# gaozhitong/MultiShiftSeg

Measured on AMD Instinct MI355X. Metric: train images/sec (DeepLabV3+ WRN38, fwd + RelContrastiveLoss + bwd + Adam), higher is better.
Workload: dtype f32; 1 GPU; c3: 2 images (1 orig+aug pair(s)) of 1024x2048 per GPU, stage-2 trainable set, train-mode BN/Dropout2d on the frozen trunk; images_per_gpu=2, height=1024, width=2048, stage=2, parallelism=dp1, rccl_ranks=0, loss_pairing=device, loss_sync=local

## Files before the change

multishiftseg_amd/csrc/conv_igemm.hip:

```cpp
#include "mss_epilogue.h"
#include <stdlib.h>

#include "fwd_route.h"

int mss_gemm_nt_launch(MssConvArgs p, const FwdRoute& r, void* stream);
int mss_fwd_bf16x3_launch(MssConvArgs p, const FwdRoute& r, void* stream);
int mss_stem7_launch(MssConvArgs p, void* stream);
int mss_conv_dgrad_s2_launch(MssConvArgs p, const FwdRoute& r, void* stream);

namespace {

constexpr int NT = 256;

template <int BM, int BN, int BK, int WM, int WN, bool PER_SAMPLE, bool AFFINE>
__global__ __launch_bounds__(NT) void conv_igemm_kernel(MssConvArgs p) {
  constexpr int LDK = BK + 4;
  constexpr int WTM = BM / WM, WTN = BN / WN;
  constexpr int TM = WTM / 32, TN = WTN / 32;
  constexpr int CPR = BK / 4;
  constexpr int RPP = NT / CPR;
  constexpr int A_LD = BM / RPP, B_LD = BN / RPP;
  static_assert(WM * WN == 4, "4 waves per workgroup");
  static_assert(A_LD >= 1 && B_LD >= 1, "tile too small for 256 threads");

  extern __shared__ __attribute__((aligned(16))) float smem[];
  int* live_mask_p = reinterpret_cast<int*>(smem);
  float* As = smem + 4;
  float* Bs = As + 2 * BM * LDK;

  const int tid = threadIdx.x;
  const int lane = tid & 63;
  const int wave = tid >> 6;
  const int wm = wave / WN, wn = wave % WN;

  p.x += (size_t)blockIdx.y * p.x_bs;
  p.w += (size_t)blockIdx.y * p.w_bs;
  p.y += (size_t)blockIdx.y * p.y_bs;
  const int v = mss_xcd_remap(blockIdx.x, gridDim.x);
  const int mt = v / p.ntiles, nt = v % p.ntiles;
  const int m0 = mt * BM, n0 = nt * BN;

  const int chunk = tid % CPR;
  const int row0 = tid / CPR;

  int a_nb[A_LD], a_iy0[A_LD], a_ix0[A_LD], a_n[A_LD];
  const int ohw = p.OH * p.OW;
  int my_live = 0;
  if (tid == 0) *live_mask_p = 0;
#pragma unroll
  for (int j = 0; j < A_LD; ++j) {
    int m = m0 + row0 + j * RPP;
    if (m < p.M) {
      int n = m / ohw, rem = m - n * ohw;
      int oy = rem / p.OW, ox = rem - oy * p.OW;
      a_n[j] = n;
      a_nb[j] = n * p.H * p.W;
      a_iy0[j] = oy * p.stride - p.pad;
      a_ix0[j] = ox * p.stride - p.pad;
      for (int t = 0; t < p.R * p.S; ++t) {
        int iy = a_iy0[j] + (t / p.S) * p.dil, ix = a_ix0[j] + (t % p.S) * p.dil;
        if ((unsigned)iy < (unsigned)p.H && (unsigned)ix < (unsigned)p.W) my_live |= 1 << t;
      }
    } else {
      a_n[j] = 0; a_nb[j] = 0; a_iy0[j] = -0x40000000; a_ix0[j] = -0x40000000;
    }
  }
  __syncthreads();
  if (my_live) atomicOr(live_mask_p, my_live);
  __syncthreads();
  const int live = *live_mask_p;
  const int nlive = __popc(live);
  const int cblocks = p.C / BK;
  const int n_it = nlive * cblocks;

  f32x16 acc[TM][TN];
#pragma unroll
  for (int i = 0; i < TM; ++i)
#pragma unroll
    for (int j = 0; j < TN; ++j)
#pragma unroll
      for (int r = 0; r < 16; ++r) acc[i][j][r] = 0.f;

  constexpr int S_LD = 1;
  f32x4 areg[A_LD], breg[B_LD], sreg[S_LD], hreg[S_LD];
  const float* a_ptr[A_LD];
  const float* b_ptr[B_LD];
  const float* s_ptr[S_LD];
  const float* h_ptr[S_LD];
  unsigned a_ok = 0;
  unsigned ld_ok = 0;
  int ld_cc = 0;
  int ld_tap = -1, ld_c0 = 0, ld_left = live;
  constexpr bool has_affine = AFFINE;
  const float relu_floor = p.in_relu ? 0.f : -__builtin_huge_valf();

  auto next_tap = [&]() {
    ld_tap = __ffs(ld_left) - 1;
    ld_left &= ld_left - 1;
    ld_c0 = 0;
    const int r = ld_tap / p.S, s = ld_tap - r * p.S;
    const int dy = r * p.dil, dx = s * p.dil;
    a_ok = 0;
#pragma unroll
    for (int j = 0; j < A_LD; ++j) {
      const int iy = a_iy0[j] + dy, ix = a_ix0[j] + dx;
      const bool ok = (unsigned)iy < (unsigned)p.H && (unsigned)ix < (unsigned)p.W;
      a_ok |= (ok ? 1u : 0u) << j;
      a_ptr[j] = ok ? p.x + (size_t)(a_nb[j] + iy * p.W + ix) * p.ldx + chunk * 4 : p.x;
    }
#pragma unroll
    for (int j = 0; j < B_LD; ++j)
      b_ptr[j] = p.w + ((size_t)ld_tap * p.Kpad + n0 + row0 + j * RPP) * p.C + chunk * 4;
    if (has_affine) {
#pragma unroll
      for (int j = 0; j < S_LD; ++j) {
        const size_t so = (size_t)(m0 / ohw) * p.in_ss_stride + chunk * 4;
        s_ptr[j] = p.in_scale + so;
        h_ptr[j] = p.in_shift + so;
      }
    }
  };

  auto issue_loads = [&]() {
#pragma unroll
    for (int j = 0; j < A_LD; ++j) areg[j] = *reinterpret_cast<const f32x4*>(a_ptr[j]);
#pragma unroll
    for (int j = 0; j < B_LD; ++j) breg[j] = *reinterpret_cast<const f32x4*>(b_ptr[j]);
    if (has_affine) {
#pragma unroll
      for (int j = 0; j < S_LD; ++j) {
        sreg[j] = *reinterpret_cast<const f32x4*>(s_ptr[j]);
        hreg[j] = *reinterpret_cast<const f32x4*>(h_ptr[j]);
      }
    }
    ld_cc = ld_c0 + chunk * 4;
    ld_ok = a_ok;
  };
  auto advance = [&]() {
    if (ld_c0 + BK >= p.C) {
      if (ld_left) next_tap();
    } else {
      ld_c0 += BK;
#pragma unroll
      for (int j = 0; j < A_LD; ++j)
        if ((a_ok >> j) & 1) a_ptr[j] += BK;
#pragma unroll
      for (int j = 0; j < B_LD; ++j) b_ptr[j] += BK;
      if (has_affine) {
#pragma unroll
        for (int j = 0; j < S_LD; ++j) { s_ptr[j] += BK; h_ptr[j] += BK; }
      }
    }
  };

  auto finish_store = [&](int buf) {
#pragma unroll
    for (int j = 0; j < A_LD; ++j) {
      f32x4 val = areg[j];
      if (has_affine) {
        if (PER_SAMPLE) {
          const size_t so = (size_t)a_n[j] * p.in_ss_stride + ld_cc;
          val = val * *reinterpret_cast<const f32x4*>(p.in_scale + so) + *reinterpret_cast<const f32x4*>(p.in_shift + so);
        } else {
          val = val * sreg[0] + hreg[0];
        }
      }
      val.x = fmaxf(val.x, relu_floor); val.y = fmaxf(val.y, relu_floor);
      val.z = fmaxf(val.z, relu_floor); val.w = fmaxf(val.w, relu_floor);
      if (!((ld_ok >> j) & 1)) val = f32x4{0.f, 0.f, 0.f, 0.f};
      *reinterpret_cast<f32x4*>(&As[(buf * BM + row0 + j * RPP) * LDK + chunk * 4]) = val;
    }
#pragma unroll
    for (int j = 0; j < B_LD; ++j)
      *reinterpret_cast<f32x4*>(&Bs[(buf * BN + row0 + j * RPP) * LDK + chunk * 4]) = breg[j];
  };

  if (n_it > 0) {
    next_tap();
    issue_loads();
    finish_store(0);
    advance();
    issue_loads();
    advance();
  }
  __syncthreads();

  constexpr int NKC = BK / 8;
  const int frag_row = lane & 31, frag_k = (lane >> 5) * 4;
  const float* Abase = &As[(wm * WTM + frag_row) * LDK + frag_k];
  const float* Bbase = &Bs[(wn * WTN + frag_row) * LDK + frag_k];
  f32x4 fa[2][TM], fb[2][TN];
  auto load_frags = [&](int set, int buf, int kc) {
#pragma unroll
    for (int i = 0; i < TM; ++i)
      fa[set][i] = *reinterpret_cast<const f32x4*>(Abase + (buf * BM + i * 32) * LDK + kc * 8);
#pragma unroll
    for (int j = 0; j < TN; ++j)
      fb[set][j] = *reinterpret_cast<const f32x4*>(Bbase + (buf * BN + j * 32) * LDK + kc * 8);
  };
  auto mfma_chunk = [&](int set) {
#pragma unroll
    for (int s = 0; s < 4; ++s)
#pragma unroll
      for (int i = 0; i < TM; ++i)
#pragma unroll
        for (int j = 0; j < TN; ++j)
          acc[i][j] = __builtin_amdgcn_mfma_f32_32x32x2f32(fa[set][i][s], fb[set][j][s], acc[i][j], 0, 0, 0);
  };

  if (n_it > 0) load_frags(0, 0, 0);
  for (int it = 0; it < n_it; ++it) {
    const int buf = it & 1;
#pragma unroll
    for (int kc = 0; kc < NKC; ++kc) {
      if (kc + 1 < NKC) load_frags((kc + 1) & 1, buf, kc + 1);
      if (kc == NKC - 2) { finish_store(buf ^ 1); issue_loads(); advance(); }
      if (kc == NKC - 1) {
        __syncthreads();
        load_frags(NKC & 1, buf ^ 1, 0);
      }
      mfma_chunk(kc & 1);
    }
  }

  mss_epilogue_store<TM, TN>(acc, p, p.y, m0 + wm * WTM, n0 + wn * WTN, lane);
}

template <int BM, int BN, int BK, int WM, int WN, bool PS, bool AFF>
int launch_conv_t(const MssConvArgs& p, hipStream_t stream) {
  const size_t smem = ((size_t)2 * (BM + BN) * (BK + 4) + 4) * sizeof(float);
  constexpr auto kern = conv_igemm_kernel<BM, BN, BK, WM, WN, PS, AFF>;
  if (int rc = mss_kernel_info<kern>(NT, smem)) return rc;
  hipLaunchKernelGGL(kern, dim3(p.mtiles * p.ntiles, p.batch > 1 ? p.batch : 1), dim3(NT), smem, stream, p);
  return mss_launch_status();
}

template <int BM, int BN, int BK, int WM, int WN>
int launch_conv_tile(const MssConvArgs& p, const FwdRoute& r, hipStream_t stream) {
  if (!r.affine) return launch_conv_t<BM, BN, BK, WM, WN, false, false>(p, stream);
  return r.per_sample ? launch_conv_t<BM, BN, BK, WM, WN, true, true>(p, stream) : launch_conv_t<BM, BN, BK, WM, WN, false, true>(p, stream);
}
int launch_conv(const MssConvArgs& p, const FwdRoute& r, hipStream_t stream) {
  if (r.BN == 64) return launch_conv_tile<256, 64, 16, 4, 1>(p, r, stream);
  return r.BK == 32 ? launch_conv_tile<128, 128, 32, 2, 2>(p, r, stream) : launch_conv_tile<128, 128, 16, 2, 2>(p, r, stream);
}

__global__ void pack_weights_kernel(const float* __restrict__ src, float* __restrict__ dst, int K, int C,
                                    int R, int S, int Kpad, int Cp, int flip, const int* __restrict__ col, int n_img, int c0) {
  const size_t total = (size_t)R * S * Kpad * Cp;
  for (size_t i = blockIdx.x * (size_t)blockDim.x + threadIdx.x; i < total;
       i += (size_t)gridDim.x * blockDim.x) {
    int c = i % Cp;
    int k = (i / Cp) % Kpad;
    int t = i / ((size_t)Cp * Kpad);
    int r = t / S, s = t % S;
    float val = 0.f;
    if (col) {
      if (k < K && c < C)
        for (int n = 0; n < n_img; ++n) {
          const int cc = c < c0 ? c : col[(size_t)n * (C - c0) + c - c0];
          if (cc >= 0) val += src[((((size_t)n * K + k) * C + (c < c0 ? c : c0 + cc)) * R + r) * S + s];
        }
    } else if (!flip) {
      if (k < K && c < C) val = src[(((size_t)k * C + c) * R + r) * S + s];
    } else {
      if (k < C && c < K) val = src[(((size_t)c * C + k) * R + (R - 1 - r)) * S + (S - 1 - s)];
    }
    dst[i] = val;
  }
}

__global__ void unpack_wgrad_kernel(const float* __restrict__ src, float* __restrict__ dst, int K, int C,
                                    int R, int S, int Kpad, int Cp, int accumulate, const int* __restrict__ place,
                                    const int* __restrict__ k_steps, int n_img, int c0) {
  if (place) {
    const size_t per = (size_t)K * C * R * S, all = per * n_img;
    for (size_t i = blockIdx.x * (size_t)blockDim.x + threadIdx.x; i < all; i += (size_t)gridDim.x * blockDim.x) {
      const size_t e = i % per;
      const int n = (int)(i / per);
      const int s = e % S, r = (e / S) % R;
      const int cc = (e / ((size_t)S * R)) % C, k = e / ((size_t)S * R * C);
      int c = cc;
      if (cc >= c0) {
        const int pc = cc - c0 < 16 * k_steps[n] ? place[(size_t)n * (C - c0) + cc - c0] : -1;
        c = pc >= 0 ? c0 + pc : -1;
      }
      dst[i] = c >= 0 ? src[((size_t)(r * S + s) * Kpad + k) * Cp + c] : 0.f;
    }
    return;
  }
  const size_t total = (size_t)K * C * R * S;
  for (size_t i = blockIdx.x * (size_t)blockDim.x + threadIdx.x; i < total;
       i += (size_t)gridDim.x * blockDim.x) {
    int s = i % S;
    int r = (i / S) % R;
    int c = (i / ((size_t)S * R)) % C;
    int k = i / ((size_t)S * R * C);
    float val = src[((size_t)(r * S + s) * Kpad + k) * Cp + c];
    dst[i] = accumulate ? dst[i] + val : val;
  }
}

constexpr int WP_CH = 128;
constexpr int WP_MIN_C = 32;
constexpr int WP_ILP = 4;
constexpr int WP_COL_IMGS = 2;
constexpr int WP_MAX_TAPS = 121;

__host__ __device__ static inline int wp_pitch(int taps) { return WP_CH + (taps > 16 ? 1 : 4); }
static inline bool wp_by_lines(int channels, int taps) { return channels >= WP_MIN_C && taps >= 2 && taps <= WP_MAX_TAPS; }

struct WpRunIndex {
  int c, t, dc, dt, taps;
  __device__ WpRunIndex(int tid, int taps_) : c(tid / taps_), t(tid % taps_), dc(256 / taps_), dt(256 % taps_), taps(taps_) {}
  __device__ void next() {
    c += dc; t += dt;
    if (t >= taps) { t -= taps; ++c; }
  }
};

__global__ __launch_bounds__(256) void pack_weights_lines_kernel(const float* __restrict__ src, float* __restrict__ dst, int K, int C, int T,
                                                                  int Kpad, int Cp, const int* __restrict__ col, int n_img, int c0) {
  extern __shared__ float wp_tile[];
  const int chunks = (Cp + WP_CH - 1) / WP_CH, pitch = wp_pitch(T), tid = threadIdx.x;
  const int k = blockIdx.x / chunks, cb = (blockIdx.x - k * chunks) * WP_CH;
  const int nc_dst = Cp - cb < WP_CH ? Cp - cb : WP_CH;
  const int nc_src = k < K && C > cb ? (C - cb < WP_CH ? C - cb : WP_CH) : 0;
  const int run = nc_src * T;
  const float* base = src + ((size_t)(k < K ? k : 0) * C + cb) * T;
  __shared__ int wp_col[WP_COL_IMGS][WP_CH];
  auto source_channel = [&](int n, int c) {
    if (c < c0) return c;
    const int cc = col[(size_t)n * (C - c0) + c - c0];
    return cc >= 0 ? c0 + cc : -1;
  };
  if (col && run > 0) {
    for (int i = tid; i < WP_COL_IMGS * WP_CH; i += 256) {
      const int n = i / WP_CH, c = i - n * WP_CH;
      wp_col[n][c] = n < n_img && c < nc_src ? source_channel(n, cb + c) : -1;
    }
    __syncthreads();
  }
  WpRunIndex at(tid, T);
  for (int j0 = tid; j0 < run; j0 += WP_ILP * 256) {
    int cs[WP_ILP], ts[WP_ILP];
    float v[WP_ILP];
#pragma unroll
    for (int u = 0; u < WP_ILP; ++u) { cs[u] = at.c; ts[u] = at.t; at.next(); }
    if (!col) {
#pragma unroll
      for (int u = 0; u < WP_ILP; ++u) v[u] = j0 + u * 256 < run ? base[j0 + u * 256] : 0.f;
    } else {
#pragma unroll
      for (int u = 0; u < WP_ILP; ++u) v[u] = 0.f;
      for (int n = 0; n < n_img; n += 2) {
        float a[2][WP_ILP];
        bool has[2][WP_ILP];
#pragma unroll
        for (int m = 0; m < 2; ++m)
#pragma unroll
          for (int u = 0; u < WP_ILP; ++u) {
            int sc = -1;
            if (n + m < n_img && j0 + u * 256 < run) sc = n + m < WP_COL_IMGS ? wp_col[n + m][cs[u]] : source_channel(n + m, cb + cs[u]);
            has[m][u] = sc >= 0;
            a[m][u] = sc >= 0 ? src[(((size_t)(n + m) * K + k) * C + sc) * T + ts[u]] : 0.f;
          }
#pragma unroll
        for (int m = 0; m < 2; ++m)
#pragma unroll
          for (int u = 0; u < WP_ILP; ++u)
            if (has[m][u]) v[u] += a[m][u];
      }
    }
#pragma unroll
    for (int u = 0; u < WP_ILP; ++u)
      if (j0 + u * 256 < run) wp_tile[ts[u] * pitch + cs[u]] = v[u];
  }
  __syncthreads();
  const int c = tid & (WP_CH - 1);
  if (c < nc_dst)
    for (int t = tid / WP_CH; t < T; t += 256 / WP_CH)
      dst[((size_t)t * Kpad + k) * Cp + cb + c] = c < nc_src ? wp_tile[t * pitch + c] : 0.f;
}

__global__ __launch_bounds__(256) void unpack_wgrad_lines_kernel(const float* __restrict__ src, float* __restrict__ dst, int K, int C, int T,
                                                                  int Kpad, int Cp, int accumulate, const int* __restrict__ place,
                                                                  const int* __restrict__ k_steps, int c0) {
  extern __shared__ float wp_tile[];
  const int chunks = (C + WP_CH - 1) / WP_CH, pitch = wp_pitch(T), tid = threadIdx.x;
  const int nk = blockIdx.x / chunks, cb = (blockIdx.x - nk * chunks) * WP_CH;
  const int n = nk / K, k = nk - n * K;
  const int nc = C - cb < WP_CH ? C - cb : WP_CH;
  const int c = tid & (WP_CH - 1);
  if (c < nc) {
    int sc = cb + c;
    if (place && sc >= c0) {
      const int pc = sc - c0 < 16 * k_steps[n] ? place[(size_t)n * (C - c0) + sc - c0] : -1;
      sc = pc >= 0 ? c0 + pc : -1;
    }
    constexpr int DT = 256 / WP_CH;
    for (int t0 = tid / WP_CH; t0 < T; t0 += WP_ILP * DT) {
      float v[WP_ILP];
#pragma unroll
      for (int u = 0; u < WP_ILP; ++u) v[u] = sc >= 0 && t0 + u * DT < T ? src[((size_t)(t0 + u * DT) * Kpad + k) * Cp + sc] : 0.f;
#pragma unroll
      for (int u = 0; u < WP_ILP; ++u)
        if (t0 + u * DT < T) wp_tile[(t0 + u * DT) * pitch + c] = v[u];
    }
  }
  __syncthreads();
  float* base = dst + ((size_t)nk * C + cb) * T;
  const int run = nc * T;
  WpRunIndex at(tid, T);
  for (int j0 = tid; j0 < run; j0 += WP_ILP * 256) {
    float v[WP_ILP], before[WP_ILP];
#pragma unroll
    for (int u = 0; u < WP_ILP; ++u) {
      v[u] = j0 + u * 256 < run ? wp_tile[at.t * pitch + at.c] : 0.f;
      at.next();
    }
    if (accumulate) {
#pragma unroll
      for (int u = 0; u < WP_ILP; ++u) before[u] = j0 + u * 256 < run ? base[j0 + u * 256] : 0.f;
    }
#pragma unroll
    for (int u = 0; u < WP_ILP; ++u)
      if (j0 + u * 256 < run) base[j0 + u * 256] = accumulate ? before[u] + v[u] : v[u];
  }
}

}

extern "C" {

static FwdSwitches fwd_switches() {
  FwdSwitches sw;
  sw.gemm = MSS_ENV_INT("MSS_GEMM", 1);
  sw.variant = MSS_ENV_INT("MSS_GEMM_VARIANT", 3);
  sw.tail = MSS_ENV_INT("MSS_GEMM_TAIL", -1);
  sw.split_mfma = MSS_ENV_INT("MSS_GEMM_SPLIT_MFMA", 16);
  return sw;
}

int mss_conv2d_forward_f32(MssConvArgs* args, void* stream) {
  MssConvArgs p = *args;
  const FwdRoute r = fwd_route(p, fwd_switches());
  if (r.status != MSS_OK) return r.status;
  if (r.M <= 0) return MSS_OK;
  fwd_fill_args(p, r);
  switch (r.kernel) {
    case FWD_DGRAD_S2: return mss_conv_dgrad_s2_launch(p, r, stream);
    case FWD_STEM7: return mss_stem7_launch(p, stream);
    case FWD_FEW_ROWS: case FWD_GEMM_NT: case FWD_GEMM_NT_PERIMG: return mss_gemm_nt_launch(p, r, stream);
    case FWD_GEMM_NT_BF16X3: case FWD_CONV_BF16X3: case FWD_ROWAFF_BF16X3: return mss_fwd_bf16x3_launch(p, r, stream);
    default: return launch_conv(p, r, static_cast<hipStream_t>(stream));
  }
}

int mss_conv2d_forward_route(const MssConvArgs* args) { return fwd_route_code(fwd_route(*args, fwd_switches())); }

int mss_conv2d_kpad(int K) { return K <= 64 ? 64 : ((K + 127) / 128) * 128; }

int mss_conv2d_pack_weights_f32(const float* w, float* packed, int K, int C, int R, int S, int Kpad, int Cp,
                                int flip, const int* col, int n_img, int c0, void* stream) {
  if (!w || !packed) return MSS_ERR_BAD_ARG;
  if (col && (flip || n_img < 1 || c0 < 0 || c0 >= C)) return MSS_ERR_BAD_ARG;
  const long long wgs = (long long)Kpad * ((Cp + WP_CH - 1) / WP_CH);
  if (!flip && wp_by_lines(Cp, R * S) && wgs >= 1 && wgs <= 0x7fffffffll) {
    hipLaunchKernelGGL(pack_weights_lines_kernel, dim3((unsigned)wgs), dim3(256), (size_t)R * S * wp_pitch(R * S) * sizeof(float),
                       static_cast<hipStream_t>(stream), w, packed, K, C, R * S, Kpad, Cp, col, n_img, c0);
    return mss_launch_status();
  }
  const size_t total = (size_t)R * S * Kpad * Cp;
  int blocks = (int)((total + 255) / 256 < 4096 ? (total + 255) / 256 : 4096);
  hipLaunchKernelGGL(pack_weights_kernel, dim3(blocks), dim3(256), 0, static_cast<hipStream_t>(stream), w,
                     packed, K, C, R, S, Kpad, Cp, flip, col, n_img, c0);
  return mss_launch_status();
}

int mss_conv2d_unpack_wgrad_f32(const float* packed, float* grad, int K, int C, int R, int S, int Kpad, int Cp,
                                int accumulate, const int* place, const int* k_steps, int n_img, int c0, void* stream) {
  if (!grad || !packed) return MSS_ERR_BAD_ARG;
  if (place && (accumulate || !k_steps || n_img < 1 || c0 < 0 || c0 >= C)) return MSS_ERR_BAD_ARG;
  const long long wgs = (long long)(place ? n_img : 1) * K * ((C + WP_CH - 1) / WP_CH);
  if (wp_by_lines(C, R * S) && wgs >= 1 && wgs <= 0x7fffffffll) {
    hipLaunchKernelGGL(unpack_wgrad_lines_kernel, dim3((unsigned)wgs), dim3(256), (size_t)R * S * wp_pitch(R * S) * sizeof(float),
                       static_cast<hipStream_t>(stream), packed, grad, K, C, R * S, Kpad, Cp, accumulate, place, k_steps, c0);
    return mss_launch_status();
  }
  const size_t total =(size_t)K * C * R * S * (place ? n_img : 1);
  int blocks = (int)((total + 255) / 256 < 4096 ? (total + 255) / 256 : 4096);
  hipLaunchKernelGGL(unpack_wgrad_kernel, dim3(blocks), dim3(256), 0, static_cast<hipStream_t>(stream), packed,
                     grad, K, C, R, S, Kpad, Cp, accumulate, place, k_steps, n_img, c0);
  return mss_launch_status();
}

}
```

Baseline: 23.76 images/s.

## Add persistent implicit-GEMM conv kernel with cross-tile prefetch and dead-tap skipping

```diff
diff --git a/multishiftseg_amd/csrc/conv_igemm.hip b/multishiftseg_amd/csrc/conv_igemm.hip
--- a/multishiftseg_amd/csrc/conv_igemm.hip
+++ b/multishiftseg_amd/csrc/conv_igemm.hip
@@ -2,6 +2,7 @@
 #include <stdlib.h>
 
 #include "fwd_route.h"
+#include "conv_igemm_tab.h"
 
 int mss_gemm_nt_launch(MssConvArgs p, const FwdRoute& r, void* stream);
 int mss_fwd_bf16x3_launch(MssConvArgs p, const FwdRoute& r, void* stream);
@@ -226,8 +227,258 @@
   mss_epilogue_store<TM, TN>(acc, p, p.y, m0 + wm * WTM, n0 + wn * WTN, lane);
 }
 
+constexpr int IG_SLOT_FLOATS = 8;
+
+template <int BM, int BN, int BK, int WM, int WN, bool PER_SAMPLE, bool AFFINE>
+__global__ __launch_bounds__(NT, (BK == 16 && BM == 128 && !PER_SAMPLE) ? 3 : 2) void conv_igemm_kernel3(MssConvArgs p, int total_tiles, int tiles_per_batch) {
+  constexpr bool ROT = BK == 16;
+  constexpr int LDK = ROT ? BK : BK + 4;
+  constexpr int WTM = BM / WM, WTN = BN / WN;
+  constexpr int TM = WTM / 32, TN = WTN / 32;
+  constexpr int CPR = BK / 4, RPP = NT / CPR;
+  constexpr int A_LD = BM / RPP, B_LD = BN / RPP;
+  constexpr int NKC = BK / 8;
+  constexpr unsigned STEP = BK * sizeof(float);
+  static_assert(WM * WN == 4 && A_LD >= 1 && B_LD >= 1 && NKC >= 2, "4 waves, 256 threads stage whole passes");
+  static_assert(!ROT || RPP % 16 == 0, "rows of one thread share their rotation");
+
+  extern __shared__ __attribute__((aligned(16))) float smem[];
+  unsigned* slots = reinterpret_cast<unsigned*>(smem);
+  float* As = smem + IG_SLOT_FLOATS;
+  float* Bs = As + 2 * BM * LDK;
+
+  const int tid = threadIdx.x, lane = tid & 63, wave = tid >> 6;
+  const int wm = wave / WN, wn = wave % WN;
+  const int chunk = tid % CPR, row0 = tid / CPR;
+  const int wchunk = ROT ? (chunk + (row0 >> 2)) & 3 : chunk;
+  const int cblocks = p.C / BK;
+  const int stride = gridDim.x;
+  const IgGeom g = ig_geom(p);
+  const unsigned w_tap = (unsigned)((size_t)p.Kpad * p.C * sizeof(float));
+  const float relu_floor = p.in_relu ? 0.f : -__builtin_huge_valf();
+  const char* xb = reinterpret_cast<const char*>(p.x);
+  const char* wb = reinterpret_cast<const char*>(p.w);
+
+  IgLoader<A_LD> ld;
+  unsigned live_n = 0;
+  unsigned b_row[B_LD];
+#pragma unroll
+  for (int j = 0; j < B_LD; ++j) b_row[j] = (unsigned)(((size_t)(row0 + j * RPP) * p.C + chunk * 4) * sizeof(float));
+  const unsigned c_row = chunk * 16;
+  auto decode_next = [&](int t, int q) {
+    IgGeom gt = g;
+    asm volatile("" : "+s"(gt.OH), "+s"(gt.OW));
+    const int b = t / tiles_per_batch, v = t - b * tiles_per_batch;
+    const int mt = v / p.ntiles, nt = v - mt * p.ntiles;
+    const int m0 = mt * BM;
+    unsigned my_live = 0;
+#pragma unroll
+    for (int j = 0; j < A_LD; ++j) {
+      unsigned mask;
+      ig_row(gt, b, m0 + row0 + j * RPP, ld.rb_n[j], mask, ld.an_n[j]);
+      ld.rb_n[j] += chunk * 16;
+      ig_pack_mask<A_LD>(ld.mkp_n, j, mask);
+      my_live |= mask;
+    }
+    ld.bu_n = (unsigned)(((size_t)b * p.w_bs + (size_t)(nt * BN) * p.C) * sizeof(float));
+    ld.su_n = AFFINE ? (unsigned)((size_t)(m0 / (gt.OH * gt.OW)) * p.in_ss_stride * sizeof(float)) : 0u;
+#pragma unroll
+    for (int o = 32; o > 0; o >>= 1) my_live |= (unsigned)__shfl_xor((int)my_live, o);
+    if (lane == 0) slots[q * 4 + wave] = my_live;
+  };
+  auto read_live = [&](int q) {
+    const uint4 s = *reinterpret_cast<const uint4*>(slots + q * 4);
+    return (unsigned)__builtin_amdgcn_readfirstlane((int)(s.x | s.y | s.z | s.w));
+  };
+
+  auto advance = [&]() {
+    const int tap = ig_next_tap(ld, live_n, cblocks);
+    ig_advance(ld, live_n, tap, ig_tap_delta(g, tap), w_tap, cblocks, STEP);
+  };
+  f32x4 areg[A_LD], breg[B_LD], sreg, hreg;
+  unsigned st_in[IgLoader<A_LD>::NW];
+  int st_cc = 0;
+  int st_an[A_LD];
+  auto issue_loads = [&]() {
+#pragma unroll
+    for (int j = 0; j < A_LD; ++j) areg[j] = *reinterpret_cast<const f32x4*>(xb + ld.a_off[j]);
+#pragma unroll
+    for (int j = 0; j < B_LD; ++j) breg[j] = *reinterpret_cast<const f32x4*>(wb + (ld.b_off + b_row[j]));
+    if (AFFINE && !PER_SAMPLE) {
+      sreg = *reinterpret_cast<const f32x4*>(reinterpret_cast<const char*>(p.in_scale) + (ld.s_off + c_row));
+      hreg = *reinterpret_cast<const f32x4*>(reinterpret_cast<const char*>(p.in_shift) + (ld.s_off + c_row));
+    }
+#pragma unroll
+    for (int w = 0; w < IgLoader<A_LD>::NW; ++w) st_in[w] = ld.mkp[w] >> ld.tap;
+    if (PER_SAMPLE) {
+      st_cc = ld.cb * BK + chunk * 4;
+#pragma unroll
+      for (int j = 0; j < A_LD; ++j) st_an[j] = ld.an[j];
+    }
+  };
+  auto finish_store = [&](int buf) {
+#pragma unroll
+    for (int j = 0; j < A_LD; ++j) {
+      f32x4 val = areg[j];
+      if (AFFINE) {
+        if (PER_SAMPLE) {
+          const size_t so = (size_t)st_an[j] * p.in_ss_stride + st_cc;
+          val = val * *reinterpret_cast<const f32x4*>(p.in_scale + so) + *reinterpret_cast<const f32x4*>(p.in_shift + so);
+        } else {
+          val = val * sreg + hreg;
+        }
+      }
+      val.x = fmaxf(val.x, relu_floor); val.y = fmaxf(val.y, relu_floor);
+      val.z = fmaxf(val.z, relu_floor); val.w = fmaxf(val.w, relu_floor);
+      if (!ig_in(st_in[j / 3], j, 0)) val = f32x4{0.f, 0.f, 0.f, 0.f};
+      *reinterpret_cast<f32x4*>(&As[(buf * BM + row0 + j * RPP) * LDK + wchunk * 4]) = val;
+    }
+#pragma unroll
+    for (int j = 0; j < B_LD; ++j)
+      *reinterpret_cast<f32x4*>(&Bs[(buf * BN + row0 + j * RPP) * LDK + wchunk * 4]) = breg[j];
+  };
+
+  const int frag_row = lane & 31, frag_h = lane >> 5;
+  const int rot = ROT ? frag_row >> 2 : 0;
+  const float* Abase = &As[(wm * WTM + frag_row) * LDK];
+  const float* Bbase = &Bs[(wn * WTN + frag_row) * LDK];
+  int koff[NKC];
+#pragma unroll
+  for (int kc = 0; kc < NKC; ++kc) koff[kc] = ROT ? ((kc * 2 + frag_h + rot) & 3) * 4 : (kc * 2 + frag_h) * 4;
+  f32x4 fa[2][TM], fb[2][TN];
+  auto load_frags = [&](int set, int buf, int kc) {
+#pragma unroll
+    for (int i = 0; i < TM; ++i)
+      fa[set][i] = *reinterpret_cast<const f32x4*>(Abase + (buf * BM + i * 32) * LDK + koff[kc]);
+#pragma unroll
+    for (int j = 0; j < TN; ++j)
+      fb[set][j] = *reinterpret_cast<const f32x4*>(Bbase + (buf * BN + j * 32) * LDK + koff[kc]);
+  };
+  f32x16 acc[TM][TN];
+  auto zero_acc = [&]() {
+#pragma unroll
+    for (int i = 0; i < TM; ++i)
+#pragma unroll
+      for (int j = 0; j < TN; ++j)
+#pragma unroll
+        for (int r = 0; r < 16; ++r) acc[i][j][r] = 0.f;
+  };
+  auto mfma_chunk = [&](int set) {
+#pragma unroll
+    for (int s = 0; s < 4; ++s)
+#pragma unroll
+      for (int i = 0; i < TM; ++i)
+#pragma unroll
+        for (int j = 0; j < TN; ++j)
+          acc[i][j] = __builtin_amdgcn_mfma_f32_32x32x2f32(fa[set][i][s], fb[set][j][s], acc[i][j], 0, 0, 0);
+  };
+  auto epilogue = [&](int t) {
+    const int b = t / tiles_per_batch, v = t - b * tiles_per_batch;
+    const int mt = v / p.ntiles, nt = v - mt * p.ntiles;
+    int tl = tid;
+    asm volatile("" : "+v"(tl));
+    const int ew = tl >> 6;
+    mss_epilogue_store<TM, TN>(acc, p, p.y + (size_t)b * p.y_bs, mt * BM + (ew / WN) * WTM, nt * BN + (ew % WN) * WTN, tl & 63);
+  };
+
+  int rnd = 0, cur = ig_tile_at(blockIdx.x, 0, stride, total_tiles);
+  auto tile_behind = [&]() {
+    const int t = ig_tile_at(blockIdx.x, rnd + 1, stride, total_tiles);
+    return t < 0 ? cur : t;
+  };
+  decode_next(cur, 0);
+  __syncthreads();
+  live_n = read_live(0);
+  int cur_nit = __popc(live_n) * cblocks;
+  ld.left = 0; ld.cb = cblocks - 1; ld.tap = 0;
+#pragma unroll
+  for (int j = 0; j < A_LD; ++j) { ld.rb[j] = ld.a_off[j] = 0; ld.an[j] = 0; }
+#pragma unroll
+  for (int w = 0; w < IgLoader<A_LD>::NW; ++w) ld.mkp[w] = 0;
+  ld.bu = ld.b_off = ld.su = ld.s_off = 0;
+  advance();
+  int q = 1;
+  decode_next(tile_behind(), q);
+  __syncthreads();
+  live_n = read_live(q);
+  issue_loads();
+  finish_store(0);
+  advance();
+  issue_loads();
+  advance();
+  zero_acc();
+  __syncthreads();
+  load_frags(0, 0, 0);
+  int buf = 0, k = 0;
+  while (true) {
+#pragma unroll
+    for (int kc = 0; kc < NKC; ++kc) {
+      if (kc + 1 < NKC) load_frags((kc + 1) & 1, buf, kc + 1);
+      if (kc == NKC - 2) {
+        finish_store(buf ^ 1);
+        issue_loads();
+        advance();
+      }
+      if (kc == NKC - 1) {
+        __syncthreads();
+        load_frags(NKC & 1, buf ^ 1, 0);
+        live_n = read_live(q);
+      }
+      mfma_chunk(kc & 1);
+      if (NKC == 2 && kc == 0) {
+#pragma unroll
+        for (int i = 0; i < TM + TN; ++i) { __builtin_amdgcn_sched_group_barrier(0x8, 1, 0); __builtin_amdgcn_sched_group_barrier(0x100, 1, 0); }
+#pragma unroll
+        for (int i = 0; i < A_LD + B_LD; ++i) { __builtin_amdgcn_sched_group_barrier(0x8, 1, 0); __builtin_amdgcn_sched_group_barrier(0x200, 1, 0); }
+#pragma unroll
+        for (int i = 0; i < A_LD + B_LD; ++i) { __builtin_amdgcn_sched_group_barrier(0x8, 1, 0); __builtin_amdgcn_sched_group_barrier(0x20, 1, 0); }
+#pragma unroll
+        for (int i = 0; i < 4 * TM * TN - (TM + TN) - 2 * (A_LD + B_LD); ++i) { __builtin_amdgcn_sched_group_barrier(0x8, 1, 0); __builtin_amdgcn_sched_group_barrier(0x6, 2, 0); }
+      }
+    }
+    buf ^= 1;
+    if (++k == cur_nit) {
+      epilogue(cur);
+      cur = ig_tile_at(blockIdx.x, ++rnd, stride, total_tiles);
+      if (cur < 0) break;
+      zero_acc();
+      k = 0;
+      cur_nit = __popc(live_n) * cblocks;
+      q ^= 1;
+      decode_next(tile_behind(), q);
+    }
+  }
+}
+
+template <int BM, int BN, int BK, bool PS, bool AFF>
+constexpr bool ig_loop3_built() { return BM == 128 && BK == 16 && !PS; }
+
+struct IgLaunch { int grid, slots, total, tiles_per_batch; size_t smem; };
+template <int BM, int BN, int BK, int WM, int WN, bool PS, bool AFF>
+int ig_launch_plan(const MssConvArgs& p, IgLaunch& l) {
+  l = IgLaunch{0, 0, 0, 0, 0};
+  if (!ig_loop3_built<BM, BN, BK, PS, AFF>() || !ig_loop3_ok(p, BK, MSS_ENV_INT("MSS_GEMM_VARIANT", 3))) return MSS_OK;
+  l.smem = ((size_t)2 * (BM + BN) * (BK == 16 ? BK : BK + 4) + IG_SLOT_FLOATS) * sizeof(float);
+  MssKernelInfo ki;
+  if (int rc = mss_kernel_info<conv_igemm_kernel3<BM, BN, BK, WM, WN, PS, AFF>>(NT, l.smem, 1, &ki)) return rc;
+  l.tiles_per_batch = p.mtiles * p.ntiles;
+  l.total = l.tiles_per_batch * (p.batch > 1 ? p.batch : 1);
+  l.slots = ki.occ * ki.cus;
+  const int cap = MSS_ENV_INT("MSS_IGEMM_MAX_WGS", 0);
+  int grid = l.total < l.slots ? l.total : l.slots;
+  if (cap > 0 && cap < grid) grid = cap;
+  l.grid = grid < l.total ? grid : 0;
+  return MSS_OK;
+}
+
 template <int BM, int BN, int BK, int WM, int WN, bool PS, bool AFF>
 int launch_conv_t(const MssConvArgs& p, hipStream_t stream) {
+  IgLaunch l;
+  if (int rc = ig_launch_plan<BM, BN, BK, WM, WN, PS, AFF>(p, l)) return rc;
+  if (l.grid > 0) {
+    hipLaunchKernelGGL((conv_igemm_kernel3<BM, BN, BK, WM, WN, PS, AFF>), dim3(l.grid), dim3(NT), l.smem, stream, p, l.total, l.tiles_per_batch);
+    return mss_launch_status();
+  }
   const size_t smem = ((size_t)2 * (BM + BN) * (BK + 4) + 4) * sizeof(float);
   constexpr auto kern = conv_igemm_kernel<BM, BN, BK, WM, WN, PS, AFF>;
   if (int rc = mss_kernel_info<kern>(NT, smem)) return rc;
@@ -235,6 +486,13 @@
   return mss_launch_status();
 }
 
+template <int BM, int BN, int BK, int WM, int WN, bool PS, bool AFF>
+int conv_slots_t(const MssConvArgs& p, int what) {
+  IgLaunch l;
+  if (ig_launch_plan<BM, BN, BK, WM, WN, PS, AFF>(p, l)) return -1;
+  return what ? l.grid : (l.grid > 0 ? l.slots : 0);
+}
+
 template <int BM, int BN, int BK, int WM, int WN>
 int launch_conv_tile(const MssConvArgs& p, const FwdRoute& r, hipStream_t stream) {
   if (!r.affine) return launch_conv_t<BM, BN, BK, WM, WN, false, false>(p, stream);
@@ -243,6 +501,15 @@
 int launch_conv(const MssConvArgs& p, const FwdRoute& r, hipStream_t stream) {
   if (r.BN == 64) return launch_conv_tile<256, 64, 16, 4, 1>(p, r, stream);
   return r.BK == 32 ? launch_conv_tile<128, 128, 32, 2, 2>(p, r, stream) : launch_conv_tile<128, 128, 16, 2, 2>(p, r, stream);
+}
+template <int BM, int BN, int BK, int WM, int WN>
+int conv_slots_tile(const MssConvArgs& p, const FwdRoute& r, int what) {
+  if (!r.affine) return conv_slots_t<BM, BN, BK, WM, WN, false, false>(p, what);
+  return r.per_sample ? conv_slots_t<BM, BN, BK, WM, WN, true, true>(p, what) : conv_slots_t<BM, BN, BK, WM, WN, false, true>(p, what);
+}
+int conv_slots(const MssConvArgs& p, const FwdRoute& r, int what) {
+  if (r.BN == 64) return conv_slots_tile<256, 64, 16, 4, 1>(p, r, what);
+  return r.BK == 32 ? conv_slots_tile<128, 128, 32, 2, 2>(p, r, what) : conv_slots_tile<128, 128, 16, 2, 2>(p, r, what);
 }
 
 __global__ void pack_weights_kernel(const float* __restrict__ src, float* __restrict__ dst, int K, int C,
@@ -459,6 +726,14 @@
 
 int mss_conv2d_forward_route(const MssConvArgs* args) { return fwd_route_code(fwd_route(*args, fwd_switches())); }
 
+int mssi_conv2d_igemm_slots(const MssConvArgs* args, int what) {
+  MssConvArgs p = *args;
+  const FwdRoute r = fwd_route(p, fwd_switches());
+  if (r.status != MSS_OK || r.kernel != FWD_CONV_IGEMM || r.M <= 0) return -1;
+  fwd_fill_args(p, r);
+  return conv_slots(p, r, what);
+}
+
 int mss_conv2d_kpad(int K) { return K <= 64 ? 64 : ((K + 127) / 128) * 128; }
 
 int mss_conv2d_pack_weights_f32(const float* w, float* packed, int K, int C, int R, int S, int Kpad, int Cp,
diff --git a/multishiftseg_amd/csrc/conv_igemm_tab.h b/multishiftseg_amd/csrc/conv_igemm_tab.h
--- /dev/null
+++ b/multishiftseg_amd/csrc/conv_igemm_tab.h
@@ -0,0 +1,126 @@
+#pragma once
+#include "fwd_route.h"
+
+#ifdef __HIPCC__
+#define IG_HD __host__ __device__ __forceinline__
+#define IG_UNROLL _Pragma("unroll")
+#else
+#define IG_HD inline
+#define IG_UNROLL
+#endif
+
+constexpr int IG_MIN_CBLOCKS = 4;
+
+struct IgGeom {
+  int H, W, OH, OW, S, taps, stride, dil, pad, ldx, M;
+  long long x_bs;
+  unsigned s_inv, dy, dx;
+};
+
+IG_HD IgGeom ig_geom(const MssConvArgs& p) {
+  return IgGeom{p.H, p.W, p.OH, p.OW, p.S, p.R * p.S, p.stride, p.dil, p.pad, p.ldx, p.M, p.x_bs,
+                65536u / (unsigned)p.S + 1u, (unsigned)((long long)p.dil * p.W * p.ldx * 4), (unsigned)((long long)p.dil * p.ldx * 4)};
+}
+
+IG_HD int ig_xcd_remap(int bid, int nwg) {
+  const int xcd = bid & 7, q = nwg >> 3, r = nwg & 7;
+  const int base = xcd < r ? xcd * (q + 1) : r * (q + 1) + (xcd - r) * q;
+  return base + (bid >> 3);
+}
+
+IG_HD int ig_tile_at(int bid, int i, int grid, int total) {
+  const int full = total / grid, rem = total - full * grid;
+  if (i < full) return i * grid + ig_xcd_remap(bid, grid);
+  return (i == full && bid < rem) ? full * grid + ig_xcd_remap(bid, rem) : -1;
+}
+
+IG_HD void ig_row(const IgGeom& g, int b, int m, unsigned& base, unsigned& mask, int& n) {
+  base = 0; mask = 0; n = 0;
+  if (m < g.M) {
+    const int ohw = g.OH * g.OW;
+    n = m / ohw;
+    const int rem = m - n * ohw;
+    const int oy = rem / g.OW, ox = rem - oy * g.OW;
+    const int iy0 = oy * g.stride - g.pad, ix0 = ox * g.stride - g.pad;
+    for (int t = 0; t < g.taps; ++t) {
+      const int iy = iy0 + (t / g.S) * g.dil, ix = ix0 + (t % g.S) * g.dil;
+      if ((unsigned)iy < (unsigned)g.H && (unsigned)ix < (unsigned)g.W) mask |= 1u << t;
+    }
+    base = (unsigned)(((long long)b * g.x_bs + (((long long)n * g.H + iy0) * g.W + ix0) * g.ldx) * 4);
+  }
+}
+
+IG_HD unsigned ig_tap_delta(const IgGeom& g, int t) {
+  const unsigned r = ((unsigned)t * g.s_inv) >> 16, c = (unsigned)t - r * (unsigned)g.S;
+  return r * g.dy + c * g.dx;
+}
+
+template <int A_LD>
+struct IgLoader {
+  static constexpr int NW = (A_LD + 2) / 3;
+  unsigned rb[A_LD], rb_n[A_LD];
+  unsigned mkp[NW], mkp_n[NW];
+  int an[A_LD], an_n[A_LD];
+  unsigned bu, bu_n;
+  unsigned su, su_n;
+  unsigned left;
+  int tap, cb;
+  unsigned a_off[A_LD], b_off, s_off;
+};
+template <int A_LD>
+IG_HD void ig_pack_mask(unsigned (&mkp)[(A_LD + 2) / 3], int j, unsigned mask) {
+  if (j % 3 == 0) mkp[j / 3] = 0;
+  mkp[j / 3] |= mask << (9 * (j % 3));
+}
+IG_HD unsigned ig_in(unsigned word, int j, int t) { return (word >> (9 * (j % 3) + t)) & 1u; }
+
+template <int A_LD>
+IG_HD int ig_next_tap(const IgLoader<A_LD>& s, unsigned live_n, int cblocks) {
+  const unsigned left = (s.cb + 1 == cblocks && s.left == 0) ? live_n : s.left;
+  return left ? __builtin_ffs((int)left) - 1 : 0;
+}
+template <int A_LD>
+IG_HD void ig_advance(IgLoader<A_LD>& s, unsigned live_n, int tap, unsigned td, unsigned w_tap, int cblocks, unsigned step) {
+  const bool last_cb = s.cb + 1 == cblocks;
+  const bool wrap = last_cb && s.left == 0;
+  const unsigned left = wrap ? live_n : s.left;
+  const unsigned left_next = left & (left - 1);
+  unsigned was[A_LD];
+  IG_UNROLL
+  for (int j = 0; j < A_LD; ++j) was[j] = ig_in(s.mkp[j / 3], j, s.tap);
+  IG_UNROLL
+  for (int w = 0; w < IgLoader<A_LD>::NW; ++w) s.mkp[w] = wrap ? s.mkp_n[w] : s.mkp[w];
+  IG_UNROLL
+  for (int j = 0; j < A_LD; ++j) {
+    s.rb[j] = wrap ? s.rb_n[j] : s.rb[j];
+    s.an[j] = wrap ? s.an_n[j] : s.an[j];
+    const unsigned at_tap = (s.rb[j] + td) & (0u - ig_in(s.mkp[j / 3], j, tap));
+    const unsigned at_block = s.a_off[j] + (step & (0u - was[j]));
+    s.a_off[j] = last_cb ? at_tap : at_block;
+  }
+  s.bu = wrap ? s.bu_n : s.bu;
+  s.su = wrap ? s.su_n : s.su;
+  const unsigned b_tap = s.bu + (unsigned)tap * w_tap, b_block = s.b_off + step, s_block = s.s_off + step;
+  const int cb_next = s.cb + 1;
+  s.b_off = last_cb ? b_tap : b_block;
+  s.s_off = last_cb ? s.su : s_block;
+  s.left = last_cb ? left_next : s.left;
+  s.tap = last_cb ? tap : s.tap;
+  s.cb = last_cb ? 0 : cb_next;
+}
+
+static inline bool ig_loop3_ok(const MssConvArgs& p, int BK, int variant) {
+  if (variant != 3 || p.C / BK < IG_MIN_CBLOCKS) return false;
+  auto centre = [&](int taps, int in, int out) {
+    for (int r = 0; r < taps; ++r)
+      if (r * p.dil - p.pad >= 0 && (long long)(out - 1) * p.stride + r * p.dil - p.pad < in) return true;
+    return false;
+  };
+  if (p.stride < 1 || p.dil < 1 || !centre(p.R, p.H, p.OH) || !centre(p.S, p.W, p.OW)) return false;
+  if (p.x_bs < 0 || p.w_bs < 0 || p.in_ss_stride < 0) return false;
+  if ((long long)p.mtiles * p.ntiles * fwd_batch(p) > 0x7fffffffll || p.M > 0x7fffffff - 512) return false;
+  if (fwd_span32(fwd_batch(p), p.x_bs, (unsigned long long)p.N * p.H * p.W * p.ldx, 4, 0xffffffffull)) return false;
+  if (fwd_span32(fwd_batch(p), p.w_bs, (unsigned long long)p.R * p.S * p.Kpad * p.C, 4, 0xffffffffull)) return false;
+  if (p.in_scale && fwd_span32(p.N > 1 ? p.N : 1, p.in_ss_stride, (unsigned long long)p.C, 4, 0xffffffffull)) return false;
+  return true;
+}
```

Result: no change. 23.78 images/s (median of 3 runs) (+0.1%).
